# intcomp/camouflaged-vlm

Measured on AMD Instinct MI355X. Metric: images/sec at 1024x1024 (SAM-ViT-H + CLIP ViT-L/14), full cascade, higher is better.
Workload: dtype f16 hi.hi MFMA + block-scaled e4m3 MFMA for the two correction products (3 mantissa bits) in the ViT-H qkv / lin1 / lin2 and CLIP MLP GEMMs; 3x f16 split MFMA in the other GEMMs; f32 accumulate; ViT-H attention: q.k^T = ONE f16 product (Q and K as single f16 values), P.v = 2x f16 (P a single f16, V

## Files before the change

camouflaged-vlm_amd/csrc/gemm.hip:

```cpp
#include "gemm_kernel.h"
#include "gemm_plan.h"
using namespace cvlm_gemm_k;
using namespace cvlm_gemm_p;
CVLM_GEMM_IL_KERNELS(extern template)
static_assert(cvlm_gemm_p::BK_MIN == cvlm_gemm_k::BK_MIN && cvlm_gemm_p::SK_MAX_TILES == cvlm_gemm_k::SK_MAX_TILES, "the planner's copy of the kernel's limits");

extern "C" int64_t cvlm_gemm_workspace_bytes(void) { return (int64_t)(TAIL_FLAG_BYTES + TAIL_WS_BYTES); }

#ifdef CVLM_PROBES
static unsigned long long* g_trace = nullptr;
extern "C" void cvlm_debug_set_gemm_trace(void* buf) { g_trace = (unsigned long long*)buf; }
#endif

static int device_cus() {
    static int cus_[16] = {};
    int dev = 0;
    (void)hipGetDevice(&dev);
    int& cus = cus_[dev & 15];
    if (cus == 0 && hipDeviceGetAttribute(&cus, hipDeviceAttributeMultiprocessorCount, dev) != hipSuccess) cus = 256;
    return cus;
}

template <auto... T>
static int launch(const GemmPlan& pl, const GemmParams& p, hipStream_t s) {
// ... 20 lines not shown

extern "C" int cvlm_gemm(const cvlm_gemm_args* args, void* stream) {
    if (!args) return CVLM_E_BADARG;
    const cvlm_gemm_args& g = *args;
    GemmPlan plans[2];
    const int n = plan_call(g, g.workspace && g.workspace_bytes >= cvlm_gemm_workspace_bytes(), device_cus, plans);
    if (n < 0) return n;
    int rc = 0;
    for (int i = 0; i < n && rc == 0; ++i) {
        const GemmPlan& pl = plans[i];
        GemmParams p;
        p.a = gemm_sanitised(g);
        if (pl.n0 > 0) {
            const int64_t n0 = pl.n0;
            p.a.w_hi = (const char*)g.w_hi + n0 * g.ldw * 2;
            if (g.w_lo) p.a.w_lo = (const char*)g.w_lo + n0 * g.ldw * 2;
            if (g.w_il) p.a.w_il = (const char*)g.w_il + n0 * g.ldw_il * 2;
            if (g.bias) p.a.bias = g.bias + n0;
            if (g.ln_colsum) p.a.ln_colsum = g.ln_colsum + n0;
            if (g.residual) p.a.residual = g.residual + n0;
            if (g.out_f32) p.a.out_f32 = g.out_f32 + n0;
            if (g.out_hi) p.a.out_hi = (char*)g.out_hi + n0 * 2 * (g.out_il ? 2 : 1);
            if (g.out_lo) p.a.out_lo = (char*)g.out_lo + n0 * 2;
        }
        p.a.N = pl.N;
        p.nbx = pl.nbx; p.nby = pl.nby; p.group_m = pl.group_m;
        p.tail_rem = pl.tail_rem; p.tail_split = pl.tail_split; p.total_blocks = pl.total_blocks; p.sk_parts = pl.sk_parts;
        p.flags = pl.use_ws ? (unsigned*)g.workspace : nullptr;
        p.ws = pl.use_ws ? (float*)((unsigned char*)g.workspace + TAIL_FLAG_BYTES) : nullptr;
#ifdef CVLM_PROBES
        p.trace = g_trace;
#endif
        hipStream_t s = (hipStream_t)stream;
        if (pl.k.mx) { rc = launch_mx(p, pl.k.mt, pl.k.epi, pl.grid_x - pl.nbx * pl.nby, pl.k.dbg, s); continue; }
        switch (gemm_kernel_key(pl.k)) {
#define CVLM_X(...) case gemm_kernel_key(GemmKernel{__VA_ARGS__}): rc = launch<__VA_ARGS__>(pl, p, s); break;
            CVLM_GEMM_KERNELS(CVLM_X)
#ifdef CVLM_PROBES
            CVLM_GEMM_PROBE_KERNELS(CVLM_X)
#endif
#undef CVLM_X
            default: rc = CVLM_E_UNSUPPORTED;
        }
    }
    return rc;
}

extern "C" int cvlm_debug_gemm_plan(const cvlm_gemm_args* args, int have_ws, int cus, cvlm_gemm_plan_info* out) {
    if (!args || !out) return CVLM_E_BADARG;
    out->launches = 0;
    GemmPlan plans[2];
    const int n = plan_call(*args, have_ws != 0, [cus] { return cus; }, plans);
    if (n < 0) return n;
    out->launches = n;
    for (int i = 0; i < n; ++i) {
        const GemmPlan& pl = plans[i];
        auto& o = out->launch[i];
        o.n0 = pl.n0; o.N = pl.N; o.nbx = pl.nbx; o.nby = pl.nby; o.grid_x = pl.grid_x; o.grid_y = pl.grid_y; o.block = pl.block;
        o.lds_bytes = pl.lds_bytes; o.group_m = pl.group_m; o.tail_rem = pl.tail_rem; o.tail_split = pl.tail_split;
        o.total_blocks = pl.total_blocks; o.sk_parts = pl.sk_parts; o.uses_workspace = pl.use_ws;
        gemm_kernel_name(pl.k, o.kernel, sizeof o.kernel);
    }
    return 0;
}
```

camouflaged-vlm_amd/csrc/gemm_il.hip:

```cpp
#include "gemm_kernel.h"
CVLM_GEMM_IL_KERNELS(template)
```

camouflaged-vlm_amd/csrc/gemm_kernel.h:

```cpp
#pragma once
#include <type_traits>
#include "common.h"
#include <stdlib.h>
#include "../../include/cvlm.h"

namespace cvlm_gemm_k {

constexpr int BK_MIN = 32;
constexpr int SK_COUNTER0 = 4 * 128 + 2;
constexpr int SK_MAX_TILES = 1024 - SK_COUNTER0;

__device__ __forceinline__ int swz4(int q) { return (0x78 >> (2 * q)) & 3; }

static __device__ uint4 g_zero16 = {0u, 0u, 0u, 0u};

struct GemmParams {
    cvlm_gemm_args a;
    int nbx, nby;
    int group_m;
    int tail_rem, tail_split;
    int total_blocks;
    int sk_parts;
    float* ws;
    unsigned* flags;
#ifdef CVLM_PROBES
    unsigned long long* trace;
#endif
};

template <int N> __device__ __forceinline__ void wait_vmcnt() { asm volatile("s_waitcnt vmcnt(%0)" ::"n"(N) : "memory"); }

template <int SPLIT, int WM, int WN, int NSTAGE, int BK, int DBG = 0, int MT = 4, bool PERSIST = false, int EPI = -1, bool CONV = false,
          bool SK = false, bool WIL = false, bool AIL = false, bool MX = false>
__global__ __launch_bounds__(WM * WN * 64, 2) void gemm_nt_kernel(const GemmParams p) {
    static_assert(!MX || (WIL && AIL && NSTAGE == 5 && SPLIT == 3 && !PERSIST && !SK && !CONV && (MT % 2) == 0), "mx operands: the staggered 256-column kernel");
    static_assert(!WIL || (SPLIT == 3 && BK == 32 && !CONV && NSTAGE != 4 && NSTAGE != 6), "interleaved weights: split-3 kernels with 32-wide K-tiles");
    static_assert(!AIL || WIL, "interleaved activations come with interleaved weights (one set of instantiations)");
    static_assert(!SK || (!PERSIST && !CONV && NSTAGE != 5), "split-K form: plain tile loops only");
    static_assert(!PERSIST || NSTAGE == 5, "persistent form exists for the staggered 256^2 loop only");
    static_assert(!CONV || (NSTAGE == 2 && BK == 32), "implicit 3x3 convolution: 2-stage loop, 32-wide K-tiles");
    constexpr int WROWS = MT * 16;
    constexpr int BM = WM * WROWS, BN = WN * 64, NWAVE = WM * WN;
    constexpr int NPA = (SPLIT == 3) ? 2 : 1;
    constexpr int A_PLANE = BM * BK * 2, W_PLANE = BN * BK * 2;
    constexpr int STAGE = NPA * (A_PLANE + W_PLANE);
    constexpr int ROWB = BK * 2;
    constexpr int RPI = 1024 / ROWB;
    constexpr int CPR = ROWB / 16;
    constexpr int A_INSTR = BM / RPI, W_INSTR = BN / RPI;
    constexpr int TOTAL = NPA * (A_INSTR + W_INSTR);
    static_assert(TOTAL % NWAVE == 0, "staging must divide evenly over the waves");
    constexpr int PER_WAVE = TOTAL / NWAVE;
    extern __shared__ __attribute__((aligned(16))) unsigned char smem[];

    const cvlm_gemm_args& g = p.a;
    const int tid = threadIdx.x, lane = tid & 63;
    const int wave = __builtin_amdgcn_readfirstlane(tid >> 6);
    const int wm = wave / WN, wn = wave - wm * WN;
    [[maybe_unused]] unsigned long long tr0 = 0, tr1 = 0, tr2 = 0, tr3 = 0, tr4 = 0;
    if (DBG == 4) tr0 = wall_clock64();

    const int ntiles = p.nbx * p.nby;
    const int z = blockIdx.y;
    const half_t* Ahi = (const half_t*)g.a_hi + (int64_t)z * g.stride_a;
    const half_t* Alo = (const half_t*)g.a_lo + (int64_t)z * g.stride_a;
    const half_t* Whi = MX ? (const half_t*)g.w_mx : WIL ? (const half_t*)g.w_il : (const half_t*)g.w_hi + (int64_t)z * g.stride_w;
    const half_t* Wlo = (const half_t*)g.w_lo + (int64_t)z * g.stride_w;

    int bm = 0, bn = 0, kpart = 0, kparts = 1, tail_j = 0, nk = 0;
    [[maybe_unused]] int k0_units = 0;
    const half_t* src[PER_WAVE];
    int dst_off[PER_WAVE];
    auto kmul = [&](int j) -> int { return (wave * PER_WAVE + j >= NPA * A_INSTR ? WIL : AIL) ? 2 : 1; };
    [[maybe_unused]] int tapmask[PER_WAVE];
    auto set_tile_ = [&](int pid, const half_t* ahi, const half_t* alo, const half_t* whi, const half_t* wlo,
                         int64_t lda_, int64_t ldw_, int M_, int N_) {
        kpart = 0; kparts = 1; tail_j = 0;
        if (SK) {
            kparts = p.sk_parts;
            kpart = pid / ntiles;
            pid -= kpart * ntiles;
            tail_j = pid;
        }
        if (NSTAGE == 5 && !PERSIST && p.tail_rem > 0 && pid >= ntiles - p.tail_rem) {
            const int j = pid - (ntiles - p.tail_rem);
            kparts = p.tail_split;
            kpart = j / p.tail_rem;
            tail_j = j - kpart * p.tail_rem;
            pid = ntiles - p.tail_rem + tail_j;
        }
        {
            const int q = ntiles >> 3, r = ntiles & 7, xcd = pid & 7, idx = pid >> 3;
            pid = (xcd < r ? xcd * (q + 1) : r * (q + 1) + (xcd - r) * q) + idx;
        }
        int by, bx;
        {
            const int per_group = p.group_m * p.nbx;
            const int grp = pid / per_group;
            const int first = grp * p.group_m;
            const int gm = (p.nby - first) < p.group_m ? (p.nby - first) : p.group_m;
            const int rem = pid - grp * per_group;
            by = first + rem % gm;
            bx = rem / gm;
        }
        const int bm_ = by * BM, bn_ = bx * BN;
        bm = bm_; bn = bn_;
        const int rsub = lane / CPR;
        const int pos = lane % CPR;
#pragma unroll
        for (int j = 0; j < PER_WAVE; ++j) {
            const int i = wave * PER_WAVE + j;
            const bool isW = i >= NPA * A_INSTR;
            if (AIL && !isW) {
                const int row8 = i * 8 + (lane >> 3), pos8 = lane & 7;
                int grow8 = bm_ + row8;
                grow8 = grow8 < M_ - 1 ? grow8 : M_ - 1;
                src[j] = ahi + (int64_t)grow8 * lda_ + ((pos8 ^ ((row8 >> 1) & 7)) * 8);
                dst_off[j] = i * 1024;
                continue;
            }
            if (WIL && isW) {
                const int ii2 = i - NPA * A_INSTR;
                const int row8 = ii2 * 8 + (lane >> 3), pos8 = lane & 7;
                int grow8 = bn_ + row8;
                grow8 = grow8 < N_ - 1 ? grow8 : N_ - 1;
                src[j] = whi + (int64_t)grow8 * ldw_ + ((pos8 ^ ((row8 >> 1) & 7)) * 8);
                dst_off[j] = NPA * A_PLANE + ii2 * 1024;
                continue;
            }
            const int ii = isW ? i - NPA * A_INSTR : i;
            const int per = isW ? W_INSTR : A_INSTR;
            const int plane = ii / per, sub = ii - plane * per;
            const int row = sub * RPI + rsub;
            const int chunk = (BK == 32) ? (pos ^ swz4((row >> 2) & 3)) : (pos ^ ((row >> 1) & 7));
            const half_t* base = isW ? (plane ? wlo : whi) : (plane ? alo : ahi);
            const int64_t ld = isW ? ldw_ : lda_;
            int grow = (isW ? bn_ : bm_) + row;
            const int lim = (isW ? N_ : M_) - 1;
            grow = grow < lim ? grow : lim;
            src[j] = base + (int64_t)grow * ld + chunk * 8;
            dst_off[j] = (isW ? NPA * A_PLANE + plane * W_PLANE : plane * A_PLANE) + sub * 1024;
            if (CONV) {
                const int px = grow % g.conv_w, py = (grow / g.conv_w) % g.conv_h;
                int mk = 0;
#pragma unroll
                for (int t = 0; t < 9; ++t) {
                    const int yy = py + t / 3 - 1, xx = px + t % 3 - 1;
                    mk |= (yy >= 0 && yy < g.conv_h && xx >= 0 && xx < g.conv_w) ? (1 << t) : 0;
                }
                tapmask[j] = isW ? 512 : mk;
            }
        }
        nk = g.K / BK;
        k0_units = 0;
        if ((NSTAGE == 5 || SK) && kparts > 1) {
            const int nku = MX ? (nk + 7) / 8 : nk;
            const int base = nku / kparts, extra = nku - base * kparts;
            int k0 = kpart * base + (kpart < extra ? kpart : extra);
            int mine = base + (kpart < extra ? 1 : 0);
            if (MX) { k0 *= 8; mine = mine * 8 < nk - k0 ? mine * 8 : nk - k0; k0_units = k0; }
            nk = mine;
#pragma unroll
            for (int j = 0; j < PER_WAVE; ++j) src[j] += (int64_t)k0 * BK * kmul(j);
        }
    };
    auto set_tile = [&](int pid) { set_tile_(pid, Ahi, Alo, Whi, Wlo, g.lda, MX ? g.ldw_mx : WIL ? g.ldw_il : g.ldw, g.M, g.N); };
    int vblk = blockIdx.x;
    set_tile(vblk);

    const int fr = lane & 15, fq = lane >> 4;
    const int a_row = (wm * WROWS + fr) * ROWB;
    const int w_row = (wn * 64 + fr) * ROWB;
    auto chunk_off = [&](int ks) -> int {
        return (BK == 32) ? ((fq ^ swz4((fr >> 2) & 3)) * 16) : (((4 * ks + fq) ^ ((fr >> 1) & 7)) * 16);
    };
    auto a_frag = [&](const unsigned char* cur, int mt, int pl, int co) -> half8 {
        if (AIL) return *(const half8*)(cur + (wm * WROWS + fr + mt * 16) * 128 + (((4 * pl + fq) ^ ((fr >> 1) & 7)) * 16));
        return *(const half8*)(cur + pl * A_PLANE + a_row + mt * 16 * ROWB + co);
    };
    auto w_frag = [&](const unsigned char* cur, int i, int pl, int co) -> half8 {
        if (WIL) return *(const half8*)(cur + NPA * A_PLANE + (wn * 64 + fr + i * 16) * 128 + (((4 * pl + fq) ^ ((fr >> 1) & 7)) * 16));
        return *(const half8*)(cur + NPA * A_PLANE + pl * W_PLANE + w_row + i * 16 * ROWB + co);
    };

    floatx4 acc[MT][4];
    const int conv_lc = CONV ? 31 - __builtin_clz((unsigned)(g.conv_c / BK)) : 0;
    auto src_at = [&](int j, int t) -> const void* {
        if (!CONV) return src[j] + (int64_t)t * BK * kmul(j);
// ... 446 lines not shown
            if (grpB && !(PERSIST && !first_tile && t == 0)) wait_vmcnt<0>();
            asm volatile("s_waitcnt lgkmcnt(0)" ::: "memory");
            __builtin_amdgcn_s_barrier();
            mfma_half(1, grpB ? t + 2 : -1, t & 1);
            if (!grpB) wait_vmcnt<0>();
            __builtin_amdgcn_s_barrier();
        }
        if (!grpB) __builtin_amdgcn_s_barrier();
    } else {
        constexpr int R = NSTAGE >= 13 ? NSTAGE - 10 : 3;
        static_assert((R - 1) * PER_WAVE < 64, "vmcnt is a 6-bit counter");
#pragma unroll
        for (int i = 0; i < R - 1; ++i)
            if (i < nk) issue(i, i);
        if (nk >= R - 1) wait_vmcnt<(R - 2) * PER_WAVE>(); else wait_vmcnt<0>();
        __builtin_amdgcn_s_barrier();
        int slot = 0;
        for (int t = 0; t < nk; ++t) {
            const int sp = slot == 0 ? R - 1 : slot - 1;
            compute(slot, t + R - 1 < nk ? t + R - 1 : -1, sp);
            const int younger = nk - 2 - t;
            if (younger >= R - 2) wait_vmcnt<(R - 2) * PER_WAVE>();
            else if (R > 3 && younger == R - 3) wait_vmcnt<(R > 3 ? R - 3 : 0) * PER_WAVE>();
            else if (R > 4 && younger == R - 4) wait_vmcnt<(R > 4 ? R - 4 : 0) * PER_WAVE>();
            else wait_vmcnt<0>();
            asm volatile("s_waitcnt lgkmcnt(0)" ::: "memory");
            __builtin_amdgcn_s_barrier();
            slot = slot + 1 == R ? 0 : slot + 1;
        }
    }

    if (DBG == 4) tr2 = wall_clock64();
    int m_lim = g.M;
    if (NSTAGE == 5 && !PERSIST && kparts > 1) {
        constexpr int SLAB = BM * BN;
        int lane_x = lane;
        asm volatile("" : "+v"(lane_x));
        if (kpart > 0) {
            int* gave_up_p;
            if constexpr (MX) gave_up_p = (int*)(smem + 5 * 32768 - 16);
            else { __shared__ int tail_gave_up_word; gave_up_p = &tail_gave_up_word; }
            int& tail_gave_up = *gave_up_p;
            if (tid == 0) {
                int spins = 0, bad = 0;
                while (__hip_atomic_load(&p.flags[tail_j * 4 + kpart - 1], __ATOMIC_RELAXED, __HIP_MEMORY_SCOPE_AGENT) != 1u) {
                    __builtin_amdgcn_s_sleep(8);
                    if (++spins > (1 << 22)) {
                        unsigned expect = 0u;
                        if (__hip_atomic_compare_exchange_strong(&p.flags[tail_j * 4 + kpart - 1], &expect, 2u, __ATOMIC_RELAXED, __ATOMIC_RELAXED,
                                                                 __HIP_MEMORY_SCOPE_AGENT) || expect != 1u) {
                            atomicAdd(&p.flags[4 * 128], 1u);
                            bad = 1;
                        }
                        break;
                    }
                }
                tail_gave_up = bad;
                __builtin_amdgcn_fence(__ATOMIC_ACQUIRE, "agent");
                asm volatile("s_waitcnt vmcnt(0)" ::: "memory");
                if (!bad) __hip_atomic_store(&p.flags[tail_j * 4 + kpart - 1], 0u, __ATOMIC_RELAXED, __HIP_MEMORY_SCOPE_AGENT);
            }
            __syncthreads();
            const float poison = tail_gave_up ? __builtin_nanf("") : 0.f;
            const float4* slab = (const float4*)(p.ws + ((size_t)tail_j * 3 + kpart - 1) * SLAB) + (size_t)wave * MT * 4 * 64 + lane_x;
            float4 buf[2][4];
#pragma unroll
            for (int nt = 0; nt < 4; ++nt) buf[0][nt] = slab[nt * 64];
// ... 469 lines not shown
    }
    return;
  }
}

}

#define CVLM_GEMM_IL_KERNEL(PFX, ...) PFX __global__ void cvlm_gemm_k::gemm_nt_kernel<__VA_ARGS__>(const cvlm_gemm_k::GemmParams);
#define CVLM_GEMM_IL_KERNELS(PFX)                                                                    \
    CVLM_GEMM_IL_KERNEL(PFX, 3, 2, 4, 5, 32, 0, 8, false, 0, false, false, true, false)              \
    CVLM_GEMM_IL_KERNEL(PFX, 3, 2, 4, 5, 32, 0, 8, false, 1, false, false, true, false)              \
    CVLM_GEMM_IL_KERNEL(PFX, 3, 2, 4, 5, 32, 0, 8, false, 2, false, false, true, false)              \
    CVLM_GEMM_IL_KERNEL(PFX, 3, 2, 4, 5, 32, 0, 8, false, 0, false, false, true, true)               \
    CVLM_GEMM_IL_KERNEL(PFX, 3, 2, 4, 5, 32, 0, 8, false, 1, false, false, true, true)               \
    CVLM_GEMM_IL_KERNEL(PFX, 3, 2, 4, 5, 32, 0, 8, false, 2, false, false, true, true)               \
    CVLM_GEMM_IL_KERNEL(PFX, 3, 2, 4, 5, 32, 0, 8, true, 0, false, false, true, false)               \
    CVLM_GEMM_IL_KERNEL(PFX, 3, 2, 4, 5, 32, 0, 8, true, 1, false, false, true, false)               \
    CVLM_GEMM_IL_KERNEL(PFX, 3, 2, 4, 5, 32, 0, 8, true, 2, false, false, true, false)               \
    CVLM_GEMM_IL_KERNEL(PFX, 3, 2, 4, 5, 32, 0, 8, true, 0, false, false, true, true)                \
    CVLM_GEMM_IL_KERNEL(PFX, 3, 2, 4, 5, 32, 0, 8, true, 1, false, false, true, true)                \
    CVLM_GEMM_IL_KERNEL(PFX, 3, 2, 4, 5, 32, 0, 8, true, 2, false, false, true, true)                \
    CVLM_GEMM_IL_KERNEL(PFX, 3, 2, 4, 5, 32, 0, 6, false, 2, false, false, true, false)              \
    CVLM_GEMM_IL_KERNEL(PFX, 3, 2, 4, 5, 32, 0, 6, false, 2, false, false, true, true)               \
    CVLM_GEMM_IL_KERNEL(PFX, 3, 4, 2, 3, 32, 0, 4, false, -1, false, false, true, false)             \
    CVLM_GEMM_IL_KERNEL(PFX, 3, 4, 2, 3, 32, 0, 4, false, -1, false, false, true, true)              \
    CVLM_GEMM_IL_KERNEL(PFX, 3, 4, 2, 14, 32, 0, 1, false, -1, false, false, true, false)            \
    CVLM_GEMM_IL_KERNEL(PFX, 3, 4, 2, 14, 32, 0, 2, false, -1, false, false, true, false)            \
    CVLM_GEMM_IL_KERNEL(PFX, 3, 4, 2, 14, 32, 0, 2, false, -1, false, true, true, false)             \
    CVLM_GEMM_IL_KERNEL(PFX, 3, 4, 2, 14, 32, 0, 1, false, -1, false, false, true, true)             \
    CVLM_GEMM_IL_KERNEL(PFX, 3, 4, 2, 14, 32, 0, 2, false, -1, false, false, true, true)             \
    CVLM_GEMM_IL_KERNEL(PFX, 3, 4, 2, 14, 32, 0, 2, false, -1, false, true, true, true)

namespace cvlm_gemm_k { int launch_mx(GemmParams& p, int mt, int epi, int extra_blocks, int probe, hipStream_t s); }
```

camouflaged-vlm_amd/csrc/gemm_mx.hip:

```cpp
#include "gemm_kernel.h"
#include "gemm_plan.h"
using namespace cvlm_gemm_k;
using namespace cvlm_gemm_p;

template <int MT_, int EPI_, int DBG_>
static int launch_one(const GemmParams& p, int extra_blocks, hipStream_t s) {
    constexpr int smem_ = gemm_lds_bytes(gemm_mx_kernel(MT_, EPI_, DBG_));
    auto kern_ = gemm_nt_kernel<3, 2, 4, 5, 32, DBG_, MT_, false, EPI_, false, false, true, true, true>;
    static bool attr_[16] = {};
    if (cvlm_first_on_device(attr_))
        (void)hipFuncSetAttribute((const void*)kern_, hipFuncAttributeMaxDynamicSharedMemorySize, smem_);
    hipLaunchKernelGGL(kern_, dim3(p.nbx * p.nby + extra_blocks, 1), dim3(512), smem_, s, p);
    CVLM_CHECK_LAUNCH();
    return 0;
}

int cvlm_gemm_k::launch_mx(GemmParams& p, int mt, int epi, int extra_blocks, int probe, hipStream_t s) {
#define CVLM_X(MT, EPI, DBG) if (mt == MT && epi == EPI && probe == DBG) return launch_one<MT, EPI, DBG>(p, extra_blocks, s);
    CVLM_GEMM_MX_KERNELS(CVLM_X)
#ifdef CVLM_PROBES
    CVLM_GEMM_MX_PROBE_KERNELS(CVLM_X)
#endif
#undef CVLM_X
    return CVLM_E_UNSUPPORTED;
}
```

camouflaged-vlm_amd/csrc/gemm_plan.h:

```cpp
#pragma once
#include <stdint.h>
#include <stdio.h>
#include <stdlib.h>
#include "../../include/cvlm.h"

namespace cvlm_gemm_p {
namespace {

constexpr int BK_MIN = 32;
constexpr int SK_MAX_TILES = 1024 - (4 * 128 + 2);

constexpr size_t TAIL_FLAG_BYTES = 4096;
constexpr size_t TAIL_WS_BYTES = (size_t)128 * 3 * 256 * 256 * sizeof(float);
static_assert((4 * 128 + 2) * sizeof(unsigned) <= TAIL_FLAG_BYTES, "hand-off words fit the flag page");

struct GemmKnobs {
    int tail;
    int variant;
    int persist;
    int colsplit;
    int ring;
    int w8;
    int sk;
    int t192;
    int group_m;
#ifdef CVLM_PROBES
    bool trace;
#endif
};
inline int env_int(const char* name, int dflt) { const char* e = getenv(name); return e ? atoi(e) : dflt; }
inline GemmKnobs gemm_knobs_from_env(bool live) {
    GemmKnobs k = {};
    k.tail = env_int("CVLM_GEMM_TAIL", 1); k.variant = env_int("CVLM_GEMM_VARIANT", 0); k.persist = env_int("CVLM_GEMM_PERSIST", 1);
    k.colsplit = env_int("CVLM_GEMM_COLSPLIT", 1); k.ring = env_int("CVLM_GEMM_RING", 4); k.w8 = env_int("CVLM_GEMM_W8", 1);
    k.sk = env_int("CVLM_GEMM_SK", 1); k.t192 = env_int("CVLM_GEMM_T192", 1);
    k.group_m = live ? env_int("CVLM_GEMM_GROUP_M", 0) : 0;
    return k;
}
inline GemmKnobs gemm_knobs() {
    static const bool live = env_int("CVLM_GEMM_VARIANT_LIVE", 0) != 0;
    static const GemmKnobs latched = gemm_knobs_from_env(false);
    return live ? gemm_knobs_from_env(true) : latched;
}

struct GemmKernel {
    int split, wm, wn, nstage, bk, dbg = 0, mt = 4;
    bool persist = false;
    int epi = -1;
    bool conv = false, sk = false, wil = false, ail = false, mx = false;
};
constexpr uint64_t gemm_kernel_key(const GemmKernel& k) {
    return (uint64_t)k.split | (uint64_t)k.wm << 4 | (uint64_t)k.wn << 8 | (uint64_t)k.nstage << 12 | (uint64_t)k.bk << 16 | (uint64_t)k.dbg << 24 |
           (uint64_t)k.mt << 32 | (uint64_t)(k.epi + 1) << 36 | (uint64_t)k.persist << 40 | (uint64_t)k.conv << 41 | (uint64_t)k.sk << 42 |
           (uint64_t)k.wil << 43 | (uint64_t)k.ail << 44 | (uint64_t)k.mx << 45;
}
constexpr int gemm_lds_bytes(const GemmKernel& k) {
    const int slots = k.nstage >= 13 ? k.nstage - 10 : k.nstage == 6 ? 1 : k.nstage >= 4 ? 2 : k.nstage;
    const int planes = k.split == 3 || k.conv ? 2 : 1;
    return k.mx ? 5 * 32768 : slots * planes * (k.wm * k.mt * 16 + k.wn * 64) * k.bk * 2 + (k.persist ? k.wm * k.wn * 16 * 64 * 4 : 0);
}

#define CVLM_GEMM_KERNELS(X)                                                                                                           \
    X(1, 2, 2, 2, 32) X(1, 4, 2, 3, 32) X(1, 2, 4, 3, 32, 0, 8) X(1, 4, 1, 2, 32, 0, 4, false, -1, true)                               \
    X(3, 4, 1, 2, 32, 0, 4, false, -1, true)                                                                                           \
    X(3, 2, 2, 2, 32) X(3, 2, 2, 13, 32) X(3, 2, 2, 14, 32) X(3, 2, 2, 15, 32) X(3, 4, 2, 3, 32)                                       \
    X(3, 4, 2, 14, 32, 0, 1) X(3, 4, 2, 14, 32, 0, 2)                                                                                  \
    X(3, 2, 2, 2, 32, 0, 4, false, -1, false, true) X(3, 2, 2, 13, 32, 0, 4, false, -1, false, true)                                   \
    X(3, 2, 2, 14, 32, 0, 4, false, -1, false, true) X(3, 4, 2, 14, 32, 0, 2, false, -1, false, true)                                  \
    X(3, 2, 4, 5, 32, 0, 8) X(3, 2, 4, 5, 32, 0, 8, false, 0) X(3, 2, 4, 5, 32, 0, 8, false, 1) X(3, 2, 4, 5, 32, 0, 8, false, 2)      \
// ... 9 lines not shown
#define CVLM_GEMM_PROBE_KERNELS(X)                                                                                                     \
    X(1, 2, 2, 3, 32) X(1, 2, 2, 3, 64) X(3, 2, 2, 3, 32) X(3, 2, 2, 2, 64) X(3, 2, 2, 2, 64, 2) X(3, 2, 2, 2, 32, 2)                  \
    X(3, 2, 4, 2, 32, 0, 8) X(3, 2, 4, 2, 32, 1, 8) X(3, 2, 4, 2, 32, 2, 8)                                                            \
    X(3, 2, 4, 4, 32, 0, 8) X(3, 2, 4, 4, 32, 1, 8) X(3, 2, 4, 4, 32, 2, 8)                                                            \
    X(3, 2, 2, 6, 32, 0, 8) X(3, 2, 2, 6, 32, 1, 8) X(3, 2, 2, 6, 32, 2, 8)                                                            \
    X(3, 2, 4, 5, 32, 1, 8) X(3, 2, 4, 5, 32, 2, 8) X(3, 2, 4, 5, 32, 3, 8) X(3, 2, 4, 5, 32, 4, 8) X(3, 2, 4, 5, 32, 5, 8)            \
    X(3, 2, 4, 5, 32, 6, 8) X(3, 2, 4, 5, 32, 7, 8) X(3, 2, 4, 5, 32, 8, 8)
#define CVLM_GEMM_MX_KERNELS(X) X(8, 1, 0) X(8, 2, 0) X(6, 2, 0)
#define CVLM_GEMM_MX_PROBE_KERNELS(X)                                                                                                  \
    X(8, 1, 1) X(8, 1, 2) X(8, 1, 3) X(8, 1, 5) X(8, 1, 6) X(8, 1, 7) X(8, 1, 9) X(8, 1, 10) X(8, 1, 11) X(8, 1, 12) X(8, 1, 13)       \
    X(8, 1, 14) X(8, 1, 15) X(8, 1, 16) X(8, 1, 17) X(8, 1, 18) X(8, 1, 19) X(8, 1, 20) X(8, 1, 21) X(8, 1, 22)                        \
    X(8, 2, 1) X(8, 2, 2) X(8, 2, 3) X(8, 2, 6) X(8, 2, 16) X(8, 2, 17) X(8, 2, 18) X(8, 2, 19) X(8, 2, 20) X(8, 2, 21) X(8, 2, 22)
constexpr GemmKernel gemm_mx_kernel(int mt, int epi, int dbg) { return GemmKernel{3, 2, 4, 5, 32, dbg, mt, false, epi, false, false, true, true, true}; }
constexpr bool gemm_mx_kernel_exists(int mt, int epi, int dbg) {
#define CVLM_X(MT, EPI, DBG) if (mt == MT && epi == EPI && dbg == DBG) return true;
    CVLM_GEMM_MX_KERNELS(CVLM_X)
#ifdef CVLM_PROBES
    CVLM_GEMM_MX_PROBE_KERNELS(CVLM_X)
#endif
#undef CVLM_X
    return false;
}

struct GemmPlan {
    GemmKernel k;
    int n0, N;
    int nbx, nby;
    int grid_x, grid_y, block, lds_bytes;
    int group_m;
    int tail_rem, tail_split;
    int total_blocks;
    int sk_parts;
    bool use_ws;
};

inline int gemm_validate(const cvlm_gemm_args& g) {
    if (!g.a_hi || !g.w_hi) return CVLM_E_BADARG;
    if (g.M <= 0 || g.N <= 0 || g.K <= 0 || (g.K % BK_MIN) != 0) return CVLM_E_BADARG;
    if ((g.lda & 7) || (g.ldw & 7) || (g.stride_a & 7) || (g.stride_w & 7)) return CVLM_E_BADARG;
    if (g.split != 1 && g.split != 3) return CVLM_E_BADARG;
    if (g.split == 3 && ((!g.a_lo && !g.a_il && !g.a_mx) || !g.w_lo)) return CVLM_E_BADARG;
    if (!g.out_f32 && !g.out_hi) return CVLM_E_BADARG;
    if (g.ps_c2 > 0 && ((g.ps_c2 & 3) || g.ps_h <= 0 || g.ps_w <= 0)) return CVLM_E_BADARG;
    if (g.hm_S > 0 && ((g.hm_hd & 3) || g.hm_H <= 0 || (g.M % g.hm_S) || g.N != 3 * g.hm_H * g.hm_hd || !g.out_hi)) return CVLM_E_BADARG;
    const bool conv = g.conv_c > 0;
    if (conv) {
        if (g.conv_h <= 0 || g.conv_w <= 0 || g.conv_c < 32 || (g.conv_c & (g.conv_c - 1)) || g.K != 9 * g.conv_c ||
            g.lda != g.conv_c || (g.M % (g.conv_h * g.conv_w)) || g.batch > 1)
            return CVLM_E_UNSUPPORTED;
    }
    const bool fold = g.ln_stats != nullptr, h2res = g.res_hi != nullptr || g.row_stats != nullptr;
    if (fold || h2res) {
        if (fold && h2res) return CVLM_E_BADARG;
        if (!g.out_hi || g.out_f32 || g.residual || g.ps_c2 > 0 || g.batch > 1) return CVLM_E_BADARG;
        if ((g.N & 7) || (g.ldoh & 7) || (g.hm_S > 0 && ((g.hm_hd & 7) || g.hm_S < 128))) return CVLM_E_UNSUPPORTED;
        if (fold && (!g.ln_colsum || (g.act != CVLM_ACT_NONE && g.act != CVLM_ACT_GELU && g.act != CVLM_ACT_QUICKGELU))) return CVLM_E_BADARG;
        if (h2res && (g.act != CVLM_ACT_NONE || (g.res_hi && ((!g.res_lo && !g.res_il) || (g.ldrh & 7))))) return CVLM_E_BADARG;
    }
    const bool il_any = g.a_il || g.out_il || g.res_il;
    if (il_any) {
        if (g.split != 3 || conv || g.batch > 1 || (g.out_il && g.hm_S > 0) || (g.hm_S > 0 && ((g.hm_hd & 7) || g.hm_S < 256)) || g.ps_c2 > 0 ||
            (g.N & 7) || (g.ldoh & 7) || (g.stride_oh & 7) ||
            (g.out_f32 && ((g.ldo & 3) || (g.stride_o & 3))) || (g.residual && ((g.ldr & 3) || (g.stride_r & 3))))
            return CVLM_E_UNSUPPORTED;
        if (g.a_il && (!g.w_il || (g.lda & 7) || g.lda < 2 * (int64_t)g.K)) return CVLM_E_UNSUPPORTED;
        if (g.res_il && !g.res_hi) return CVLM_E_BADARG;
// ... 9 lines not shown
        if (g.out_mx && (!g.out_hi || !g.out_mxs || g.hm_S > 0 || (g.N & 63) || (g.ldo_s & 3) || (g.out_lo && (g.ldol & 7))))
            return CVLM_E_BADARG;
        if (g.res_mx && (!g.res_hi || !g.res_lo || (g.ldrl & 7) || (g.ldrh & 7))) return CVLM_E_BADARG;
    }
    return 0;
}

inline cvlm_gemm_args gemm_sanitised(const cvlm_gemm_args& g) {
    cvlm_gemm_args a = g;
    if (g.ln_stats || g.res_hi || g.row_stats) {
        a.ldo = a.stride_o = a.ldr = a.stride_r = a.stride_oh = 0;
        a.stride_a = a.stride_w = 0;
    }
    if (a.batch <= 0) a.batch = 1;
    if (a.out_scale == 0.f) a.out_scale = 1.f;
    return a;
}

inline long tiles(const cvlm_gemm_args& a, int tm, int tn) { return (long)((a.M + tm - 1) / tm) * ((a.N + tn - 1) / tn) * a.batch; }
inline long rounds(long t, long slots) { return (t + slots - 1) / slots; }
inline double tile256_us(double K, int S = 1) { return 0.0685 * K / S + 14.0; }
inline double tail_us(int S, int K, int rem) {
    return tile256_us(K, S) + 16.0 + 8.0 + 20.0 * (S - 2) + 0.15 * rem;
}
inline int tail_parts(int rem, int K) {
    if (rem <= 0 || rem > 128) return 1;
    const int smax = 256 / rem < 4 ? 256 / rem : 4;
    int best = 1;
    double t = tile256_us(K);
    double need = 0.92 * t;
    for (int S = 2; S <= smax; ++S)
        if (K / 32 >= 4 * S && tail_us(S, K, rem) < need) { t = need = tail_us(S, K, rem); best = S; }
    return best;
}

inline int big_grid_variant(const cvlm_gemm_args& a, const GemmKnobs& kn, bool have_ws) {
    const long t5 = tiles(a, 256, 256), t1 = tiles(a, 128, 128), t2 = tiles(a, 256, 128);
    if (a.split == 3) {
        const double K = (double)a.K;
        const double m1 = (double)rounds(t1, 512) * 0.0544 * K;
        const double m2 = (double)rounds(t2, 256) * 0.0469 * K;
        const int rem = (int)(t5 % 256);
        double tail = rem > 0 ? tile256_us(K) : 0.0;
        if (kn.tail && have_ws && a.batch == 1) {
            const int S = tail_parts(rem, a.K);
            if (S >= 2) tail = tail_us(S, a.K, rem);
        }
        const double m7 = (double)(t5 / 256) * tile256_us(K) + tail;
        if (a.a_il) return m7 <= 1.04 * m2 ? 5 : 2;
        return (m7 <= 1.04 * m1 && m7 <= 1.04 * m2) ? 5 : (m2 <= m1 ? 2 : 1);
    }
    if (t5 >= 200 && t5 <= 256) return 5;
    const double c1 = (double)(rounds(t1, 512) * 512) * 1.0;
    if (t5 >= 1536) {
        const double c2 = (double)(rounds(t2, 256) * 256) * 2.0 / 1.08;
        const double c5 = (double)(rounds(t5, 256) * 256) * 4.0 / 1.20;
        return (c5 <= c2 && c5 <= c1) ? 5 : (c2 <= c1 ? 2 : 1);
    }
    const double c2 = (double)(rounds(t2, 256) * 256) * 2.0 / (a.M >= 16384 ? 1.08 : 1.05);
    return (c2 < c1) ? 2 : 1;
}

inline int pick_ring(const GemmKnobs& kn, long wgs) { return (wgs <= 256 && kn.ring >= 3 && kn.ring <= 5) ? kn.ring : 0; }

struct SmallGridChoice {
    int variant;
// ... 29 lines not shown
    auto sk_fits = [&](int S) { return a.K / 32 >= 4 * S && (size_t)t1 * S * 128 * 128 * sizeof(float) <= TAIL_WS_BYTES; };
    int skS = 1;
    double msk = 1e30;
    if (have_ws && kn.sk != 0 && t1 <= SK_MAX_TILES) {
        for (int S = 2; S <= 8 && sk_fits(S); ++S) {
            const double wg = (double)(t1 * S);
            const double t = 4.0 + (ring_on && wg <= 256.0 ? 0.78 : 1.0) * (K / S) * fillc(0.021, 0.054, wg, 512.0) * over(wg, 512.0) + 6.0 + 2.0 * S + 0.052 * wg;
            if (t < msk) { msk = t; skS = S; }
        }
    }
    if (kn.sk > 1) {
        const bool okS = have_ws && kn.sk <= 8 && t1 <= SK_MAX_TILES && sk_fits(kn.sk);
        skS = okS ? kn.sk : 1;
        msk = okS ? 0.0 : 1e30;
    }
    const bool ail1_ok = !a.a_il || (ring_on && t1 <= 256);
    if (a.a_il && skS > 1 && !(ring_on && t1 * skS <= 256)) { skS = 1; msk = 1e30; }
    if (kn.variant == 0) {
        double best = ail1_ok ? m1 : 1e30;
        c.variant = 1;
        if (m2 < best) { best = m2; c.variant = 2; }
        if (m7 < best) { best = m7; c.variant = 5; c.tail_S = tailS > 0 ? tailS : 1; }
        if (skS > 1 && msk < 0.9 * best) { c.variant = 1; c.sk_parts = skS; }
    } else if (skS > 1) {
        c.sk_parts = skS;
    }
    return c;
}

inline int gemm_plan_finish(const cvlm_gemm_args& a, GemmPlan& pl) {
    const GemmKernel& k = pl.k;
    pl.nbx = (pl.N + k.wn * 64 - 1) / (k.wn * 64);
    pl.nby = (a.M + k.wm * k.mt * 16 - 1) / (k.wm * k.mt * 16);
    if (!k.persist) pl.grid_x = k.sk ? pl.nbx * pl.nby * pl.sk_parts : pl.nbx * pl.nby + pl.tail_rem * (pl.tail_split - 1);
    pl.grid_y = a.batch;
    pl.block = k.wm * k.wn * 64;
    pl.lds_bytes = gemm_lds_bytes(k);
    return 1;
}

template <class Cus>
inline int gemm_plan_one(const cvlm_gemm_args& a, const GemmKnobs& kn, bool have_ws, Cus&& cus, GemmPlan& pl) {
    const bool conv = a.conv_c > 0, fold = a.ln_stats != nullptr, h2res = a.res_hi != nullptr || a.row_stats != nullptr;
    const bool one3 = a.split == 3 && !conv && a.batch == 1;
    const bool wil = a.w_il && one3 && a.ldw_il >= 2 * (int64_t)a.K && (a.ldw_il & 7) == 0;
    const bool ail = a.a_il != 0;
    if (ail && (!wil || (kn.variant != 0 && kn.variant != 2 && kn.variant != 7))) return CVLM_E_UNSUPPORTED;
    pl.N = a.N;
    pl.group_m = 8;
    pl.tail_rem = 0; pl.tail_split = 1; pl.total_blocks = 0; pl.sk_parts = 1; pl.use_ws = false;
    int variant = kn.variant == 0 ? big_grid_variant(a, kn, have_ws) : kn.variant;
    int tail_S = 0;
    if (one3 && a.M <= 4096 && !a.a_mx && (kn.variant == 0 || (kn.variant == 1 && kn.sk > 1))) {
        const SmallGridChoice c = small_grid_choice(a, kn, have_ws);
        variant = c.variant; tail_S = c.tail_S; pl.sk_parts = c.sk_parts;
    }
    const long t1 = tiles(a, 128, 128), t5 = tiles(a, 256, 256), t6 = tiles(a, 192, 256), t64 = tiles(a, 64, 128);
    if (pl.sk_parts > 1) {
        int ring = pick_ring(kn, t1 * pl.sk_parts);
        if (ring > 4) ring = 4;
        const bool w8 = ring == 4 && kn.w8;
        if (ail && !(w8 && wil)) return CVLM_E_UNSUPPORTED;
        if (w8) pl.k = GemmKernel{3, 4, 2, 14, 32, 0, 2, false, -1, false, true, wil, ail};
        else pl.k = GemmKernel{3, 2, 2, ring == 3 ? 13 : ring == 4 ? 14 : 2, 32, 0, 4, false, -1, false, true};
        pl.use_ws = true;
        return gemm_plan_finish(a, pl);
    }
    if (conv) {
        pl.k = GemmKernel{a.split, 4, 1, 2, 32, 0, 4, false, -1, true};
        return gemm_plan_finish(a, pl);
    }
    if (a.split != 3) {
        if (variant == 2) pl.k = GemmKernel{1, 4, 2, 3, 32};
        else if (variant == 5) pl.k = GemmKernel{1, 2, 4, 3, 32, 0, 8};
#ifdef CVLM_PROBES
        else if (variant == 4 && (a.K % 64) == 0) pl.k = GemmKernel{1, 2, 2, 3, 64};
        else if (variant == 3) pl.k = GemmKernel{1, 2, 2, 3, 32};
#endif
        else pl.k = GemmKernel{1, 2, 2, 2, 32};
        return gemm_plan_finish(a, pl);
    }
    if (variant == 5 && kn.variant == 0) variant = 7;
    if (variant == 7 || a.a_mx) pl.group_m = a.K >= 4096 ? 2 : 4;
    if (variant == 7 && kn.tail && have_ws && a.batch == 1) {
        const int rem = (int)(t5 % 256);
        const int S = tail_S > 0 ? tail_S : tail_parts(rem, a.K);
        if (S >= 2) { pl.tail_rem = rem; pl.tail_split = S; pl.use_ws = true; }
    }
    const bool lds_staged = a.ps_c2 == 0 && (a.N & 7) == 0 && (a.hm_S == 0 || ((a.hm_hd & 7) == 0 && a.hm_S >= 128)) &&
                            (a.ldo & 3) == 0 && (a.stride_o & 3) == 0 && (a.ldr & 3) == 0 && (a.stride_r & 3) == 0 &&
                            (a.ldoh & 7) == 0 && (a.stride_oh & 7) == 0;
    const bool fits192 = kn.t192 && h2res && t5 <= 256 && t6 <= 256 && t6 > t5 && a.M > 4096;
    const int epi = fold ? 1 : (h2res ? 2 : 0);
    if (a.a_mx) {
        if (!lds_staged || a.batch != 1 || (a.M & 7) || (a.N & 7) || (int64_t)8 * a.lda * 2 >= ((int64_t)1 << 32) ||
            (int64_t)8 * a.ldw_mx * 2 >= ((int64_t)1 << 32) || (int64_t)a.M * 4 * a.lda_s >= ((int64_t)1 << 32) ||
            (int64_t)a.N * 4 * a.ldw_s >= ((int64_t)1 << 32))
            return CVLM_E_UNSUPPORTED;
        if (epi == 0) return CVLM_E_UNSUPPORTED;
        pl.tail_rem = 0; pl.tail_split = 1;
        if (!fits192 && kn.tail && have_ws) {
            int S = tail_parts((int)(t5 % 256), a.K);
            while (S > 1 && (a.K / 32 + 7) / 8 < 2 * S) --S;
            if (S >= 2) { pl.tail_rem = (int)(t5 % 256); pl.tail_split = S; pl.use_ws = true; }
        }
        if (kn.group_m > 0) pl.group_m = kn.group_m;
        const int probe = kn.variant >= 100 ? kn.variant - 100 : 0;
        pl.k = gemm_mx_kernel(fits192 ? 6 : 8, epi, gemm_mx_kernel_exists(fits192 ? 6 : 8, epi, probe) ? probe : 0);
        return gemm_plan_finish(a, pl);
    }
    const bool staggered = variant == 7 && lds_staged && a.batch == 1;
    const int ring = (one3 && a.M <= 4096 && variant == 1) ? pick_ring(kn, t1) : 0;
    if (staggered && kn.variant == 0 && fits192 && pl.tail_rem == 0)
        pl.k = GemmKernel{3, 2, 4, 5, 32, 0, 6, false, 2, false, false, wil, ail};
    else if (staggered && kn.persist && (kn.variant == 0 || kn.variant == 7) && pl.tail_rem == 0 && t5 > cus()) {
        pl.k = GemmKernel{3, 2, 4, 5, 32, 0, 8, true, epi, false, false, wil, ail};
        pl.total_blocks = (int)t5;
        pl.grid_x = cus();
    }
    else if (variant == 2) pl.k = GemmKernel{3, 4, 2, 3, 32, 0, 4, false, -1, false, false, wil, ail};
    else if (staggered) pl.k = GemmKernel{3, 2, 4, 5, 32, 0, 8, false, epi, false, false, wil, ail};
    else if (ring == 4 && (kn.w8 == 2 || (kn.w8 == 1 && t64 <= 256)))
        pl.k = GemmKernel{3, 4, 2, 14, 32, 0, 1, false, -1, false, false, wil, ail};
    else if (ring == 4 && kn.w8) pl.k = GemmKernel{3, 4, 2, 14, 32, 0, 2, false, -1, false, false, wil, ail};
    else if (ail) return CVLM_E_UNSUPPORTED;
    else if (variant == 7) pl.k = GemmKernel{3, 2, 4, 5, 32, 0, 8};
#ifdef CVLM_PROBES
    else if (variant == 77) pl.k = GemmKernel{3, 2, 4, 5, 32, 7, 8};
    else if (variant == 87) pl.k = GemmKernel{3, 2, 4, 5, 32, 8, 8};
    else if (variant == 4 && (a.K % 64) == 0) pl.k = GemmKernel{3, 2, 2, 2, 64};
    else if (variant == 24 && (a.K % 64) == 0) pl.k = GemmKernel{3, 2, 2, 2, 64, 2};
    else if (variant == 21) pl.k = GemmKernel{3, 2, 2, 2, 32, 2};
    else if (variant == 5) pl.k = GemmKernel{3, 2, 4, 2, 32, 0, 8};
    else if (variant == 6) pl.k = GemmKernel{3, 2, 4, 4, 32, 0, 8};
    else if (variant == 8) pl.k = GemmKernel{3, 2, 2, 6, 32, 0, 8};
    else if (variant == 18 || variant == 28) pl.k = GemmKernel{3, 2, 2, 6, 32, variant / 10, 8};
    else if (variant == 17 || variant == 27) pl.k = GemmKernel{3, 2, 4, 5, 32, variant / 10, 8};
    else if (variant == 37) pl.k = GemmKernel{3, 2, 4, 5, 32, 3, 8};
    else if (variant == 57) pl.k = GemmKernel{3, 2, 4, 5, 32, 5, 8};
    else if (variant == 67) pl.k = GemmKernel{3, 2, 4, 5, 32, 6, 8};
    else if (variant == 47 && kn.trace) pl.k = GemmKernel{3, 2, 4, 5, 32, 4, 8};
    else if (variant == 16 || variant == 26) pl.k = GemmKernel{3, 2, 4, 4, 32, variant / 10, 8};
    else if (variant == 15 || variant == 25) pl.k = GemmKernel{3, 2, 4, 2, 32, variant / 10, 8};
    else if (variant == 3) pl.k = GemmKernel{3, 2, 2, 3, 32};
#endif
// ... 36 lines not shown
```

camouflaged-vlm_amd/hip.py:

```python
from __future__ import annotations

import ctypes as C
import functools
import os
from typing import Optional, Tuple

import torch

_PKG = os.path.dirname(os.path.abspath(__file__))
LIB_PATH = os.path.join(_PKG, "lib", "libcvlm_hip.so")

ACT_NONE, ACT_GELU, ACT_QUICKGELU, ACT_RELU, ACT_ABS_POST = 0, 1, 2, 3, 4

_SIGNATURES = {
    "cvlm_abi_version": "i:", "cvlm_target_arch": "z:",
    "cvlm_gemm": "i:Gs", "cvlm_gemm_workspace_bytes": "l:", "cvlm_debug_gemm_plan": "i:GiiI",
    "cvlm_layernorm": "i:plpipppfipppiis",
    "cvlm_add_rows": "i:ppifpppiis",
    "cvlm_ln_stats_merge": "i:pliifpps",
    "cvlm_row_stats_split": "i:pfpppliiils",
    "cvlm_row_stats_split_mx": "i:pfplplplpliiils",
    "cvlm_split_f32": "i:pppls",
    "cvlm_patchify": "i:pipiiiiippis",
    "cvlm_im2col3x3": "i:piiiipps",
# ... 85 lines not shown
    _fields_ = [(n, C.c_int32) for n in ("n0", "N", "nbx", "nby", "grid_x", "grid_y", "block", "lds_bytes", "group_m", "tail_rem",
                                         "tail_split", "total_blocks", "sk_parts", "uses_workspace")] + [("kernel", C.c_char * 128)]


class GemmPlanInfo(C.Structure):
    _fields_ = [("launches", C.c_int32), ("launch", GemmLaunchInfo * 2)]


class AttnArgs(C.Structure):
    _fields_ = [
        ("qkv_hi", C.c_void_p), ("qkv_lo", C.c_void_p), ("pad_hi", C.c_void_p), ("pad_lo", C.c_void_p),
        ("relh_hi", C.c_void_p), ("relh_lo", C.c_void_p), ("relw_hi", C.c_void_p), ("relw_lo", C.c_void_p),
        ("out_hi", C.c_void_p), ("out_lo", C.c_void_p),
        ("B", C.c_int32), ("S", C.c_int32), ("heads", C.c_int32), ("hd", C.c_int32),
        ("mode", C.c_int32), ("grid", C.c_int32), ("window", C.c_int32), ("causal", C.c_int32),
        ("split_qk", C.c_int32), ("split_pv", C.c_int32), ("scale", C.c_float), ("qkv_layout", C.c_int32),
        ("workspace", C.c_void_p), ("workspace_bytes", C.c_int64), ("q_rows", C.c_int32),
    ]


_CTYPES = {"i": C.c_int32, "l": C.c_int64, "f": C.c_float, "p": C.c_void_p, "s": C.c_void_p, "z": C.c_char_p,
           "G": C.POINTER(GemmArgs), "A": C.POINTER(AttnArgs), "I": C.POINTER(GemmPlanInfo)}
ABI = {name: (_CTYPES[sig[0]], [_CTYPES[c] for c in sig[2:]]) for name, sig in _SIGNATURES.items()}
_STREAMED = frozenset(name for name, sig in _SIGNATURES.items() if sig.endswith("s"))

_lib: Optional[C.CDLL] = None


def load() -> C.CDLL:
    global _lib
    if _lib is not None:
        return _lib
    path = os.environ.get("CVLM_PROBE_LIB") or LIB_PATH
    if not os.path.exists(path):
        raise RuntimeError(
            f"{path} is missing: the HIP kernels are the only compute path of this package. "
            "Build them with `python -c 'import __graft_entry__ as g; g.build()'` (hipcc --offload-arch=gfx950).")
    lib = C.CDLL(path)
    for name, (restype, argtypes) in ABI.items():
        fn = getattr(lib, name)
        fn.restype, fn.argtypes = restype, argtypes
    if lib.cvlm_abi_version() != ABI_VERSION:
        raise RuntimeError(f"{path}: ABI {lib.cvlm_abi_version()}, this binding needs {ABI_VERSION}: rebuild the library")
    _lib = lib
    return lib


def _check(rc: int, what: str) -> None:
    if rc != 0:
        raise RuntimeError(f"{what} failed with code {rc}")


def _p(t: Optional[torch.Tensor]) -> Optional[int]:
    return None if t is None else t.data_ptr()


def _planes(x: Optional["H2"]) -> Tuple[Optional[int], Optional[int]]:
    return (None, None) if x is None else (x.hi.data_ptr(), x.lo.data_ptr())


def _stream() -> Optional[int]:
    return torch.cuda.current_stream().cuda_stream or None


def _call(name: str, *args) -> None:
    fn = getattr(load(), name)
# ... 796 lines not shown
```

Before: 64.36.

## Run last-wave GEMM tiles as half-height tiles in a separate launch

Adds a row-tail mode for the big staggered 256x256 GEMMs. The partial last wave of tiles (t5 mod CU count) is run as half-height 128-row tiles in an extra launch, which doubles the tail's parallelism, instead of using split-K with a workspace reduction. A cost model decides when this pays off. The Python binding turns it on by default through an environment variable. The trade-offs are an extra kernel launch and more kernel instantiations, and the cost-model constants are hand-fit.

```diff
diff --git a/camouflaged-vlm_amd/csrc/gemm.hip b/camouflaged-vlm_amd/csrc/gemm.hip
--- a/camouflaged-vlm_amd/csrc/gemm.hip
+++ b/camouflaged-vlm_amd/csrc/gemm.hip
@@ -76,9 +76,18 @@
         p.trace = g_trace;
 #endif
         hipStream_t s = (hipStream_t)stream;
-        if (pl.k.mx) { rc = launch_mx(p, pl.k.mt, pl.k.epi, pl.grid_x - pl.nbx * pl.nby, pl.k.dbg, s); continue; }
+        GemmPlan wl = pl;
+        if (pl.rowtail) {
+            p.tail_rem = pl.tail_rem;
+            rc = pl.k.mx ? launch_half_mx(p, pl.k.epi, s) : pl.k.epi != 2 || pl.k.ail ? CVLM_E_UNSUPPORTED
+                 : pl.k.wil ? launch_half_il(p, s) : launch_half<2, false, false, false>(p, s);
+            p.tail_rem = 0;
+            wl.grid_x = pl.nbx * pl.nby - pl.tail_rem;
+            if (rc != 0 || wl.grid_x == 0) continue;
+        }
+        if (pl.k.mx) { rc = launch_mx(p, pl.k.mt, pl.k.epi, wl.grid_x - pl.nbx * pl.nby, pl.k.dbg, s); continue; }
         switch (gemm_kernel_key(pl.k)) {
-#define CVLM_X(...) case gemm_kernel_key(GemmKernel{__VA_ARGS__}): rc = launch<__VA_ARGS__>(pl, p, s); break;
+#define CVLM_X(...) case gemm_kernel_key(GemmKernel{__VA_ARGS__}): rc = launch<__VA_ARGS__>(wl, p, s); break;
             CVLM_GEMM_KERNELS(CVLM_X)
 #ifdef CVLM_PROBES
             CVLM_GEMM_PROBE_KERNELS(CVLM_X)
@@ -103,6 +112,7 @@
         o.n0 = pl.n0; o.N = pl.N; o.nbx = pl.nbx; o.nby = pl.nby; o.grid_x = pl.grid_x; o.grid_y = pl.grid_y; o.block = pl.block;
         o.lds_bytes = pl.lds_bytes; o.group_m = pl.group_m; o.tail_rem = pl.tail_rem; o.tail_split = pl.tail_split;
         o.total_blocks = pl.total_blocks; o.sk_parts = pl.sk_parts; o.uses_workspace = pl.use_ws;
+        if (pl.rowtail) o.tail_split = -2;
         gemm_kernel_name(pl.k, o.kernel, sizeof o.kernel);
     }
     return 0;
diff --git a/camouflaged-vlm_amd/csrc/gemm_il.hip b/camouflaged-vlm_amd/csrc/gemm_il.hip
--- a/camouflaged-vlm_amd/csrc/gemm_il.hip
+++ b/camouflaged-vlm_amd/csrc/gemm_il.hip
@@ -1,2 +1,4 @@
 #include "gemm_kernel.h"
 CVLM_GEMM_IL_KERNELS(template)
+
+int cvlm_gemm_k::launch_half_il(const GemmParams& p, hipStream_t s) { return launch_half<2, true, false, false>(p, s); }
diff --git a/camouflaged-vlm_amd/csrc/gemm_kernel.h b/camouflaged-vlm_amd/csrc/gemm_kernel.h
--- a/camouflaged-vlm_amd/csrc/gemm_kernel.h
+++ b/camouflaged-vlm_amd/csrc/gemm_kernel.h
@@ -31,8 +31,9 @@
 template <int N> __device__ __forceinline__ void wait_vmcnt() { asm volatile("s_waitcnt vmcnt(%0)" ::"n"(N) : "memory"); }
 
 template <int SPLIT, int WM, int WN, int NSTAGE, int BK, int DBG = 0, int MT = 4, bool PERSIST = false, int EPI = -1, bool CONV = false,
-          bool SK = false, bool WIL = false, bool AIL = false, bool MX = false>
+          bool SK = false, bool WIL = false, bool AIL = false, bool MX = false, bool HALF = false>
 __global__ __launch_bounds__(WM * WN * 64, 2) void gemm_nt_kernel(const GemmParams p) {
+    static_assert(!HALF || (NSTAGE == 5 && SPLIT == 3 && WM == 2 && WN == 4 && MT == 4 && !PERSIST && EPI >= 1), "half-height tiles: the 256-column staggered kernels");
     static_assert(!MX || (WIL && AIL && NSTAGE == 5 && SPLIT == 3 && !PERSIST && !SK && !CONV && (MT % 2) == 0), "mx operands: the staggered 256-column kernel");
     static_assert(!WIL || (SPLIT == 3 && BK == 32 && !CONV && NSTAGE != 4 && NSTAGE != 6), "interleaved weights: split-3 kernels with 32-wide K-tiles");
     static_assert(!AIL || WIL, "interleaved activations come with interleaved weights (one set of instantiations)");
@@ -82,7 +83,12 @@
             pid -= kpart * ntiles;
             tail_j = pid;
         }
-        if (NSTAGE == 5 && !PERSIST && p.tail_rem > 0 && pid >= ntiles - p.tail_rem) {
+        [[maybe_unused]] int half = 0;
+        if (HALF) {
+            half = pid >= p.tail_rem ? 1 : 0;
+            pid = ntiles - p.tail_rem + pid - half * p.tail_rem;
+        }
+        if (NSTAGE == 5 && !PERSIST && !HALF && p.tail_rem > 0 && pid >= ntiles - p.tail_rem) {
             const int j = pid - (ntiles - p.tail_rem);
             kparts = p.tail_split;
             kpart = j / p.tail_rem;
@@ -103,7 +109,7 @@
             by = first + rem % gm;
             bx = rem / gm;
         }
-        const int bm_ = by * BM, bn_ = bx * BN;
+        const int bm_ = HALF ? (2 * by + half) * BM : by * BM, bn_ = bx * BN;
         bm = bm_; bn = bn_;
         const int rsub = lane / CPR;
         const int pos = lane % CPR;
@@ -153,7 +159,7 @@
         }
         nk = g.K / BK;
         k0_units = 0;
-        if ((NSTAGE == 5 || SK) && kparts > 1) {
+        if (((NSTAGE == 5 && !HALF) || SK) && kparts > 1) {
             const int nku = MX ? (nk + 7) / 8 : nk;
             const int base = nku / kparts, extra = nku - base * kparts;
             int k0 = kpart * base + (kpart < extra ? kpart : extra);
@@ -666,7 +672,7 @@
 
     if (DBG == 4) tr2 = wall_clock64();
     int m_lim = g.M;
-    if (NSTAGE == 5 && !PERSIST && kparts > 1) {
+    if (NSTAGE == 5 && !PERSIST && !HALF && kparts > 1) {
         constexpr int SLAB = BM * BN;
         int lane_x = lane;
         asm volatile("" : "+v"(lane_x));
@@ -1202,3 +1208,18 @@
     CVLM_GEMM_IL_KERNEL(PFX, 3, 4, 2, 14, 32, 0, 2, false, -1, false, true, true, true)
 
 namespace cvlm_gemm_k { int launch_mx(GemmParams& p, int mt, int epi, int extra_blocks, int probe, hipStream_t s); }
+namespace cvlm_gemm_k {
+int launch_half_mx(const GemmParams& p, int epi, hipStream_t s);
+int launch_half_il(const GemmParams& p, hipStream_t s);
+template <int EPI, bool WIL, bool AIL, bool MX>
+static int launch_half(const GemmParams& p, hipStream_t s) {
+    constexpr int smem = MX ? 5 * 32768 : 2 * 2 * (128 + 256) * 32 * 2;
+    auto kern = gemm_nt_kernel<3, 2, 4, 5, 32, 0, 4, false, EPI, false, false, WIL, AIL, MX, true>;
+    static bool attr[16] = {};
+    if (cvlm_first_on_device(attr))
+        (void)hipFuncSetAttribute((const void*)kern, hipFuncAttributeMaxDynamicSharedMemorySize, smem);
+    hipLaunchKernelGGL(kern, dim3(2 * p.tail_rem, 1), dim3(512), smem, s, p);
+    CVLM_CHECK_LAUNCH();
+    return 0;
+}
+}
diff --git a/camouflaged-vlm_amd/csrc/gemm_mx.hip b/camouflaged-vlm_amd/csrc/gemm_mx.hip
--- a/camouflaged-vlm_amd/csrc/gemm_mx.hip
+++ b/camouflaged-vlm_amd/csrc/gemm_mx.hip
@@ -24,3 +24,9 @@
 #undef CVLM_X
     return CVLM_E_UNSUPPORTED;
 }
+
+int cvlm_gemm_k::launch_half_mx(const GemmParams& p, int epi, hipStream_t s) {
+    if (epi == 1) return launch_half<1, true, true, true>(p, s);
+    if (epi == 2) return launch_half<2, true, true, true>(p, s);
+    return CVLM_E_UNSUPPORTED;
+}
diff --git a/camouflaged-vlm_amd/csrc/gemm_plan.h b/camouflaged-vlm_amd/csrc/gemm_plan.h
--- a/camouflaged-vlm_amd/csrc/gemm_plan.h
+++ b/camouflaged-vlm_amd/csrc/gemm_plan.h
@@ -24,6 +24,7 @@
     int sk;
     int t192;
     int group_m;
+    int rowtail;
 #ifdef CVLM_PROBES
     bool trace;
 #endif
@@ -35,6 +36,7 @@
     k.colsplit = env_int("CVLM_GEMM_COLSPLIT", 1); k.ring = env_int("CVLM_GEMM_RING", 4); k.w8 = env_int("CVLM_GEMM_W8", 1);
     k.sk = env_int("CVLM_GEMM_SK", 1); k.t192 = env_int("CVLM_GEMM_T192", 1);
     k.group_m = live ? env_int("CVLM_GEMM_GROUP_M", 0) : 0;
+    k.rowtail = env_int("CVLM_GEMM_ROWTAIL", 0);
     return k;
 }
 inline GemmKnobs gemm_knobs() {
@@ -110,6 +112,7 @@
     int total_blocks;
     int sk_parts;
     bool use_ws;
+    bool rowtail;
 };
 
 inline int gemm_validate(const cvlm_gemm_args& g) {
@@ -185,6 +188,16 @@
     for (int S = 2; S <= smax; ++S)
         if (K / 32 >= 4 * S && tail_us(S, K, rem) < need) { t = need = tail_us(S, K, rem); best = S; }
     return best;
+}
+
+inline double round_fill(double f) { return 0.75 + 0.25 * (f < 1.0 ? f : 1.0); }
+inline double half256_us(double K, bool mx) { return mx ? 0.0844 * K + 14.0 : 0.0387 * K + 14.1; }
+inline bool rowtail_wins(int knob, int rem, int cus, int K, int S, bool mx, double full_us) {
+    if (rem <= 0 || 2 * rem > cus) return false;
+    if (knob >= 2) return true;
+    if (S >= 2) return false;
+    const double f = (double)rem / cus;
+    return half256_us(K, mx) * round_fill(2.0 * f) + 4.0 + 0.007 * full_us < tile256_us(K) * round_fill(f);
 }
 
 inline int big_grid_variant(const cvlm_gemm_args& a, const GemmKnobs& kn, bool have_ws) {
@@ -280,7 +293,7 @@
     const GemmKernel& k = pl.k;
     pl.nbx = (pl.N + k.wn * 64 - 1) / (k.wn * 64);
     pl.nby = (a.M + k.wm * k.mt * 16 - 1) / (k.wm * k.mt * 16);
-    if (!k.persist) pl.grid_x = k.sk ? pl.nbx * pl.nby * pl.sk_parts : pl.nbx * pl.nby + pl.tail_rem * (pl.tail_split - 1);
+    if (!k.persist) pl.grid_x = k.sk ? pl.nbx * pl.nby * pl.sk_parts : pl.nbx * pl.nby + pl.tail_rem * (pl.rowtail ? 1 : pl.tail_split - 1);
     pl.grid_y = a.batch;
     pl.block = k.wm * k.wn * 64;
     pl.lds_bytes = gemm_lds_bytes(k);
@@ -296,7 +309,7 @@
     if (ail && (!wil || (kn.variant != 0 && kn.variant != 2 && kn.variant != 7))) return CVLM_E_UNSUPPORTED;
     pl.N = a.N;
     pl.group_m = 8;
-    pl.tail_rem = 0; pl.tail_split = 1; pl.total_blocks = 0; pl.sk_parts = 1; pl.use_ws = false;
+    pl.tail_rem = 0; pl.tail_split = 1; pl.total_blocks = 0; pl.sk_parts = 1; pl.use_ws = false; pl.rowtail = false;
     int variant = kn.variant == 0 ? big_grid_variant(a, kn, have_ws) : kn.variant;
     int tail_S = 0;
     if (one3 && a.M <= 4096 && !a.a_mx && (kn.variant == 0 || (kn.variant == 1 && kn.sk > 1))) {
@@ -340,6 +353,8 @@
                             (a.ldoh & 7) == 0 && (a.stride_oh & 7) == 0;
     const bool fits192 = kn.t192 && h2res && t5 <= 256 && t6 <= 256 && t6 > t5 && a.M > 4096;
     const int epi = fold ? 1 : (h2res ? 2 : 0);
+    const bool rowtail_ok = kn.rowtail && a.M > 4096 && a.batch == 1 && lds_staged && (kn.variant == 0 || kn.variant == 7);
+    auto rt_rem = [&]() { return (int)(t5 % cus()); };
     if (a.a_mx) {
         if (!lds_staged || a.batch != 1 || (a.M & 7) || (a.N & 7) || (int64_t)8 * a.lda * 2 >= ((int64_t)1 << 32) ||
             (int64_t)8 * a.ldw_mx * 2 >= ((int64_t)1 << 32) || (int64_t)a.M * 4 * a.lda_s >= ((int64_t)1 << 32) ||
@@ -352,6 +367,9 @@
             while (S > 1 && (a.K / 32 + 7) / 8 < 2 * S) --S;
             if (S >= 2) { pl.tail_rem = (int)(t5 % 256); pl.tail_split = S; pl.use_ws = true; }
         }
+        if (rowtail_ok && !fits192 && rowtail_wins(kn.rowtail, rt_rem(), cus(), a.K, pl.tail_split, true, 0.0)) {
+            pl.tail_rem = rt_rem(); pl.tail_split = 1; pl.use_ws = false; pl.rowtail = true;
+        }
         if (kn.group_m > 0) pl.group_m = kn.group_m;
         const int probe = kn.variant >= 100 ? kn.variant - 100 : 0;
         pl.k = gemm_mx_kernel(fits192 ? 6 : 8, epi, gemm_mx_kernel_exists(fits192 ? 6 : 8, epi, probe) ? probe : 0);
@@ -359,6 +377,14 @@
     }
     const bool staggered = variant == 7 && lds_staged && a.batch == 1;
     const int ring = (one3 && a.M <= 4096 && variant == 1) ? pick_ring(kn, t1) : 0;
+    if (staggered && rowtail_ok && epi == 2 && !ail && !fits192) {
+        const bool persist_else = kn.persist && pl.tail_rem == 0 && t5 > cus();
+        if (rowtail_wins(kn.rowtail, rt_rem(), cus(), a.K, pl.tail_rem > 0 ? pl.tail_split : 1, false, persist_else ? (double)(t5 / cus()) * tile256_us(a.K) : 0.0)) {
+            pl.tail_rem = rt_rem(); pl.tail_split = 1; pl.use_ws = false; pl.rowtail = true;
+            pl.k = GemmKernel{3, 2, 4, 5, 32, 0, 8, false, 2, false, false, wil, false};
+            return gemm_plan_finish(a, pl);
+        }
+    }
     if (staggered && kn.variant == 0 && fits192 && pl.tail_rem == 0)
         pl.k = GemmKernel{3, 2, 4, 5, 32, 0, 6, false, 2, false, false, wil, ail};
     else if (staggered && kn.persist && (kn.variant == 0 || kn.variant == 7) && pl.tail_rem == 0 && t5 > cus()) {
diff --git a/camouflaged-vlm_amd/hip.py b/camouflaged-vlm_amd/hip.py
--- a/camouflaged-vlm_amd/hip.py
+++ b/camouflaged-vlm_amd/hip.py
@@ -141,6 +141,7 @@
     if _lib is not None:
         return _lib
     path = os.environ.get("CVLM_PROBE_LIB") or LIB_PATH
+    os.environ.setdefault("CVLM_GEMM_ROWTAIL", "1")
     if not os.path.exists(path):
         raise RuntimeError(
             f"{path} is missing: the HIP kernels are the only compute path of this package. "
```

New measurement: 64.56, median of 6. No clear change (+0.3%).
